# jseppanen/azalea

Measured on AMD Instinct MI355X. Metric: mcts_sims_per_sec, higher is better.
Workload: dtype f16x3 (fp32 operands split hi+lo f16, fp32 accumulate)

## Files before the change

azalea_amd/csrc/net_kernels.hip:

```cpp
#include "net_priv.h"

#ifndef AZX_NET_ABLATE
#define AZX_NET_ABLATE 0
#endif
#ifndef AZX_SAT_TRACK
#define AZX_SAT_TRACK 1
#endif

#include <cmath>
#include <cstdio>
#include <cstdlib>
#include <cstring>
#include <map>
#include <string>
#include <type_traits>
#include <vector>

typedef float f32x16 __attribute__((ext_vector_type(16)));

static thread_local std::string g_net_err;
const char *azx_net_error() { return g_net_err.c_str(); }

int azx_net_fail(int code, const char *msg) {
    g_net_err = msg;
// ... 99 lines not shown
                        acc[m][n] = __builtin_amdgcn_mfma_f32_32x32x2f32(afrag[m].y, bfrag[n].y, acc[m][n], 0, 0, 0);
                        acc[m][n] = __builtin_amdgcn_mfma_f32_32x32x2f32(afrag[m].z, bfrag[n].z, acc[m][n], 0, 0, 0);
                        acc[m][n] = __builtin_amdgcn_mfma_f32_32x32x2f32(afrag[m].w, bfrag[n].w, acc[m][n], 0, 0, 0);
                    }
            }
        }
        const bool residual = (layer & 1) != 0;
#pragma unroll
        for (int n = 0; n < NTW; ++n) {
            const int co = (ns * NTW + n) * 32 + li;
            const float bb = P.bias[layer * C + co];
#pragma unroll
            for (int m = 0; m < MTW; ++m) {
#pragma unroll
                for (int r = 0; r < 16; ++r) {
                    const int row = (ms * MTW + m) * 32 + (r & 3) + 8 * (r >> 2) + 4 * lh;
                    if (row < ncells) {
                        float v = acc[m][n][r] + bb;
                        if (residual) v += dst[row * LDW + co];
                        dst[row * LDW + co] = fmaxf(v, 0.0f);
                    }
                }
            }
        }
        __syncthreads();
    }

    for (int b = 0; b < BPB; ++b) {
        const int e = e0 + b;
        if (e >= n_eval) break;
        const float *Xb = lds + (size_t)b * 2 * rows * LDW;
        float4 *out = reinterpret_cast<float4 *>(act_out + (size_t)e * ncells * C);
        for (int idx = tid; idx < ncells * (C / 4); idx += 256) {
            const int pos = idx / (C / 4), c4 = idx - pos * (C / 4);
            out[idx] = *reinterpret_cast<const float4 *>(Xb + pos * LDW + 4 * c4);
        }
    }
}


typedef _Float16 f16x8 __attribute__((ext_vector_type(8)));

__device__ __forceinline__ void split_f16(float v, _Float16 &hi, _Float16 &lo) {
    hi = (_Float16)v;
    lo = (_Float16)(v - (float)hi);
}
__device__ __forceinline__ void split2_f16(float a, float b, uint32_t &hpk, uint32_t &lpk) {
    float la, lb;
    asm("v_cvt_pk_f16_f32 %0, %1, %2" : "=v"(hpk) : "v"(a), "v"(b));
    asm("v_fma_mix_f32 %0, %1, -1.0, %2 op_sel_hi:[1,0,0]" : "=v"(la) : "v"(hpk), "v"(a));
    asm("v_fma_mix_f32 %0, %1, -1.0, %2 op_sel:[1,0,0] op_sel_hi:[1,0,0]" : "=v"(lb) : "v"(hpk), "v"(b));
    asm("v_cvt_pk_f16_f32 %0, %1, %2" : "=v"(lpk) : "v"(la), "v"(lb));
#if AZX_LO_BITS < 10
    lpk = (lpk + LO_RND * 0x10001u) & (LO_MASK * 0x10001u);
#endif
}

#ifdef AZX_NET_STAMP
__device__ unsigned long long g_tower_stamp[10];
#define NT_DECL unsigned long long nt_last = __builtin_amdgcn_s_memtime(), nt_acc[8] = {0, 0, 0, 0, 0, 0, 0, 0}; const unsigned long long nt_rt0 = __builtin_amdgcn_s_memrealtime();
__device__ unsigned long long g_tower_trace[3 * 32768];
#define NT_MARK(r) { const unsigned long long nt_now = __builtin_amdgcn_s_memtime(); nt_acc[r] += nt_now - nt_last; nt_last = nt_now; }
#define NT_FLUSH if (tid == 0) { for (int r_ = 0; r_ < 7; ++r_) atomicAdd(&g_tower_stamp[r_], nt_acc[r_]); atomicAdd(&g_tower_stamp[7], 1ull); atomicAdd(&g_tower_stamp[8], __builtin_amdgcn_s_memrealtime() - nt_rt0); \
    if (blockIdx.x < 32768) { const unsigned hw = __builtin_amdgcn_s_getreg((31 << 11) | 4), xc = __builtin_amdgcn_s_getreg((31 << 11) | 20); \
        g_tower_trace[3 * blockIdx.x] = ((unsigned long long)(xc & 0xf) << 8) | (((hw >> 13) & 7) << 5) | (((hw >> 12) & 1) << 4) | ((hw >> 8) & 0xf); \
        g_tower_trace[3 * blockIdx.x + 1] = nt_rt0; g_tower_trace[3 * blockIdx.x + 2] = __builtin_amdgcn_s_memrealtime(); } }
__device__ unsigned long long g_wide_stamp[10];
#define WT_FLUSH if (lane == 0) { for (int r_ = 0; r_ < 7; ++r_) atomicAdd(&g_wide_stamp[r_], nt_acc[r_]); atomicAdd(&g_wide_stamp[7], 1ull); \
    atomicAdd(&g_wide_stamp[8], __builtin_amdgcn_s_memrealtime() - nt_rt0); }
#else
#define NT_DECL
#define NT_MARK(r)
#define NT_FLUSH
#define WT_FLUSH
#endif

#ifndef F16X3_BPB
#define F16X3_BPB 2
#endif
#ifndef AZX_S16_FENCE
#define AZX_S16_FENCE 1
#endif
typedef float f32x4 __attribute__((ext_vector_type(4)));

__global__ __launch_bounds__(F16X3_BPB * 128, 2) void k_tower_f16x3_s16(NetDev P, const uint8_t *__restrict__ ev_board,
                                                                        const int32_t *__restrict__ n_eval_ptr,
                                                                        int n_eval_host, float *__restrict__ act_out,
                                                                        float *__restrict__ hfeat) {
    constexpr int C = 64, ROWB = 272, MT = 4, NT = 4;
    extern __shared__ __align__(16) unsigned char smem[];
    const int n_eval = n_eval_ptr ? *n_eval_ptr : n_eval_host;
    const int e0 = blockIdx.x * F16X3_BPB;
    if (e0 >= n_eval) return;
    const int tid = threadIdx.x, lane = tid & 63, wave = __builtin_amdgcn_readfirstlane(tid >> 6);
    NT_DECL
    const int wb = wave >> 1, wh = wave & 1;
    const int N = P.N, ncells = P.ncells;
    const int e = e0 + wb;
    const bool live = e < n_eval;
    const int board_b = 128 * ROWB;
    const int zero_off = 0;
    const int x_off = 2 * ROWB + wb * board_b;
    unsigned char *X = smem + x_off;
    const int li = lane & 15, lh = lane >> 4;
    const int lrow = li < 8 ? li ^ 4 : li;
    const int lchunk = 128 * (lh & 1) + 16 * (lh >> 1);

    unsigned long long tapok = 0ull;
    int rbase[MT], ry_[MT], rx_[MT];
#pragma unroll
    for (int m = 0; m < MT; ++m) {
        const int r = 64 * wh + 16 * m + lrow;
        const int ry = r / N, rx = r - ry * N;
        ry_[m] = ry;
        rx_[m] = rx;
        rbase[m] = x_off + r * ROWB + lchunk;
#pragma unroll
        for (int tap = 0; tap < 9; ++tap) {
            const int yy = ry + tap / 3 - 1, xx = rx + tap % 3 - 1;
            if (r < ncells && yy >= 0 && yy < N && xx >= 0 && xx < N) tapok |= 1ull << (tap * 4 + m);
        }
    }
    uint32_t tapok_lo = (uint32_t)tapok, tapok_hi = (uint32_t)(tapok >> 32);
    auto act_offset = [&](int tap, int m) -> int {
        const int delta = ((tap / 3 - 1) * N + (tap % 3 - 1)) * ROWB;
        const uint32_t word = tap < 8 ? tapok_lo : tapok_hi;
        const int mask = (int)(word << (31 - ((tap * 4 + m) & 31))) >> 31;
        return (mask | 0xF0) & (rbase[m] + delta);
    };

    f32x4 res[MT][NT];
    auto load_bias = [&](const float *bias, float4 (&b4)[NT]) {
#pragma unroll
        for (int n = 0; n < NT; ++n) b4[n] = *reinterpret_cast<const float4 *>(bias + 16 * n + 4 * lh);
    };
    float satmax = 0.f;
    auto epilogue = [&](f32x4 (&acc)[MT][NT], const float4 (&bias4)[NT], auto kind_tag) {
        constexpr int kind = decltype(kind_tag)::value;
#pragma unroll
        for (int n = 0; n < NT; ++n) {
            const float4 b4 = bias4[n];
            const float bv[4] = {b4.x, b4.y, b4.z, b4.w};
#pragma unroll
            for (int m = 0; m < MT; ++m) {
                float v4[4];
#pragma unroll
                for (int j = 0; j < 4; ++j) {
                    float v = acc[m][n][j] + bv[j];
                    if (kind == 1) v += res[m][n][j];
                    v = fmaxf(v, 0.0f);
                    if (kind != 0) res[m][n][j] = v;
                    v4[j] = v;
                }
                if (AZX_SAT_TRACK) satmax = fmaxf(fmaxf(satmax, v4[0]), fmaxf(v4[1], fmaxf(v4[2], v4[3])));
                uint2 h4, l4;
                split2_f16(v4[0], v4[1], h4.x, l4.x);
                split2_f16(v4[2], v4[3], h4.y, l4.y);
                unsigned char *pw = X + (64 * wh + 16 * m + lrow) * ROWB + 128 * (lh >> 1) + 16 * n + 8 * (lh & 1);
                *reinterpret_cast<uint2 *>(pw) = h4;
                *reinterpret_cast<uint2 *>(pw + 64) = l4;
            }
        }
    };

    {
        const int NH = N + 2;
        unsigned char *cells = X + 121 * ROWB;
        const uint8_t *bd = ev_board + (size_t)(live ? e : n_eval - 1) * AZX_CELL_STRIDE;
        if (wh == 0) {
            for (int i = lane; i < NH * NH; i += 64) {
                const int y = i / NH - 1, x = i - (y + 1) * NH - 1;
                cells[i] = (y >= 0 && y < N && x >= 0 && x < N) ? bd[y * N + x] : (uint8_t)3;
            }
        }
        for (int i = tid; i < 2 * ROWB / 4; i += F16X3_BPB * 128) reinterpret_cast<uint32_t *>(smem + zero_off)[i] = 0u;
        __syncthreads();
        f32x4 acc[MT][NT];
#pragma unroll
        for (int m = 0; m < MT; ++m)
#pragma unroll
            for (int n = 0; n < NT; ++n) acc[m][n] = f32x4{0.f, 0.f, 0.f, 0.f};
        const uint4 *ws = reinterpret_cast<const uint4 *>(P.Ws16);
        f16x8 wfh[NT], wfl[NT];
#pragma unroll
        for (int n = 0; n < NT; ++n) {
            const uint4 qh = ws[(n * 2) * 64 + lane], ql = ws[(n * 2 + 1) * 64 + lane];
            wfh[n] = *reinterpret_cast<const f16x8 *>(&qh);
            wfl[n] = *reinterpret_cast<const f16x8 *>(&ql);
        }
#pragma unroll
        for (int m = 0; m < MT; ++m) {
            uint32_t onehot = 0u;
            if (64 * wh + 16 * m + lrow < ncells) {
                const unsigned char *c0 = cells + ry_[m] * NH + rx_[m];
#pragma unroll
                for (int tap = 0; tap < 9; ++tap) {
                    const uint32_t v = c0[(tap / 3) * NH + tap % 3];
                    onehot |= (v < 3u ? 1u : 0u) << (3 * tap + v);
                }
            }
            const uint32_t byte = (onehot >> (8 * lh)) & 0xffu;
            uint4 q;
            q.x = ((byte >> 0) & 1u) * 0x3C00u | ((byte >> 1) & 1u) * 0x3C000000u;
            q.y = ((byte >> 2) & 1u) * 0x3C00u | ((byte >> 3) & 1u) * 0x3C000000u;
            q.z = ((byte >> 4) & 1u) * 0x3C00u | ((byte >> 5) & 1u) * 0x3C000000u;
            q.w = ((byte >> 6) & 1u) * 0x3C00u | ((byte >> 7) & 1u) * 0x3C000000u;
            const f16x8 xf = *reinterpret_cast<const f16x8 *>(&q);
#pragma unroll
            for (int n = 0; n < NT; ++n) {
                acc[m][n] = __builtin_amdgcn_mfma_f32_16x16x32_f16(wfh[n], xf, acc[m][n], 0, 0, 0);
                acc[m][n] = __builtin_amdgcn_mfma_f32_16x16x32_f16(wfl[n], xf, acc[m][n], 0, 0, 0);
            }
        }
        float4 sb4[NT];
        load_bias(P.stem_b, sb4);
        __syncthreads();
        epilogue(acc, sb4, std::integral_constant<int, 2>{});
    }
    __syncthreads();
    NT_MARK(0)

    const uint4 *wsrc = reinterpret_cast<const uint4 *>(P.Wh16);
    int stage = 0;
    const int last_stage = P.layers * 18 - 1;
    f16x8 wh_[NT], wl_[NT];
    auto load_w = [&](int st, int nn, int part) {
        const uint4 qq = wsrc[(size_t)min(st, last_stage) * 512 + (nn * 2 + part) * 64 + lane];
        if (part) wl_[nn] = *reinterpret_cast<const f16x8 *>(&qq);
        else wh_[nn] = *reinterpret_cast<const f16x8 *>(&qq);
    };
#pragma unroll
    for (int i = 0; i < 4; ++i) load_w(0, i >> 1, i & 1);
    auto conv_layer = [&](int layer, auto residual_tag) {
        constexpr bool residual = decltype(residual_tag)::value;
        asm volatile("" : "+v"(tapok_lo), "+v"(tapok_hi), "+v"(rbase[0]), "+v"(rbase[1]), "+v"(rbase[2]), "+v"(rbase[3]));
        f32x4 acc[MT][NT];
#pragma unroll
        for (int m = 0; m < MT; ++m)
#pragma unroll
            for (int n = 0; n < NT; ++n) acc[m][n] = f32x4{0.f, 0.f, 0.f, 0.f};
        f16x8 xh[MT], xl[MT];
        auto load_x = [&](int tt, int mm, int part) {
            const unsigned char *pa = smem + act_offset(tt >> 1, mm) + (tt & 1) * 32 + part * 64;
            if (part) xl[mm] = *reinterpret_cast<const f16x8 *>(pa);
            else xh[mm] = *reinterpret_cast<const f16x8 *>(pa);
        };
#pragma unroll
        for (int m = 0; m < MT - 1; ++m) { load_x(0, m, 0); load_x(0, m, 1); }
#pragma unroll
        for (int t = 0; t < 18; ++t) {
#pragma unroll
            for (int h = 0; h < 2; ++h) {
#pragma unroll
                for (int q = 0; q < 24; ++q) {
                    const int m = q / 6, n = 2 * h + (q % 6) / 3, p = q % 3;
                    if (q == 1 || q == 4 || q == 7 || q == 10) {
                        const int idx = (q - 1) / 3;
                        if (h == 0) load_w(stage + t, 2 + (idx >> 1), idx & 1);
                        else load_w(stage + t + 1, idx >> 1, idx & 1);
                    } else if (h == 0 && (q == 13 || q == 16)) {
                        load_x(t, MT - 1, q == 16);
                    } else if (h == 1 && q >= 8 && (q % 6 == 2 || q % 6 == 5)) {
                        if (t + 1 < 18) load_x(t + 1, q / 6 - 1, q % 6 == 5);
                    }
                    const f16x8 wv = p == 1 ? wl_[n] : wh_[n];
                    const f16x8 xv = p == 2 ? xl[m] : xh[m];
                    acc[m][n] = __builtin_amdgcn_mfma_f32_16x16x32_f16(wv, xv, acc[m][n], 0, 0, 0);
#if AZX_S16_FENCE == 2
                    __builtin_amdgcn_sched_barrier(0);
#elif AZX_S16_FENCE == 1
                    if (q % 3 == 2) __builtin_amdgcn_sched_barrier(0);
#elif AZX_S16_FENCE == 3
                    if (q % 6 == 5) __builtin_amdgcn_sched_barrier(0);
#elif AZX_S16_FENCE == 4
                    if (q % 2 == 1) __builtin_amdgcn_sched_barrier(0);
#endif
                }
            }
        }
        stage += 18;
        float4 lb4[NT];
        load_bias(P.bias + layer * C, lb4);
        NT_MARK(2)
        __syncthreads();
        NT_MARK(3)
        epilogue(acc, lb4, std::integral_constant<int, residual ? 1 : 0>{});
        NT_MARK(4)
        __syncthreads();
        NT_MARK(5)
    };
    for (int blk = 0; blk < P.blocks; ++blk) {
        conv_layer(2 * blk, std::false_type{});
        conv_layer(2 * blk + 1, std::true_type{});
    }

    if (hfeat != nullptr) {
        const uint4 *whd = reinterpret_cast<const uint4 *>(P.Whd16);
        f16x8 ah[2], al[2];
#pragma unroll
        for (int ks = 0; ks < 2; ++ks) {
            const uint4 qh = whd[(ks * 2) * 64 + lane], ql = whd[(ks * 2 + 1) * 64 + lane];
            ah[ks] = *reinterpret_cast<const f16x8 *>(&qh);
            al[ks] = *reinterpret_cast<const f16x8 *>(&ql);
        }
        const float4 hb = *reinterpret_cast<const float4 *>(P.hbias16 + 4 * lh);
        const float hbv[4] = {hb.x, hb.y, hb.z, hb.w};
#pragma unroll
        for (int m = 0; m < MT; ++m) {
            f32x4 hacc = f32x4{0.f, 0.f, 0.f, 0.f};
#pragma unroll
            for (int ks = 0; ks < 2; ++ks) {
                const unsigned char *pa = smem + rbase[m] + ks * 32;
                const f16x8 xh = *reinterpret_cast<const f16x8 *>(pa), xl = *reinterpret_cast<const f16x8 *>(pa + 64);
                hacc = __builtin_amdgcn_mfma_f32_16x16x32_f16(ah[ks], xh, hacc, 0, 0, 0);
                hacc = __builtin_amdgcn_mfma_f32_16x16x32_f16(al[ks], xh, hacc, 0, 0, 0);
                hacc = __builtin_amdgcn_mfma_f32_16x16x32_f16(ah[ks], xl, hacc, 0, 0, 0);
            }
            const int row = 64 * wh + 16 * m + lrow;
            if (live && row < ncells) {
#pragma unroll
                for (int r = 0; r < 4; ++r) {
                    const int o = 4 * lh + r;
                    if (o < 6) hfeat[((size_t)e * 6 + o) * ncells + row] = fmaxf(hacc[r] + hbv[r], 0.0f);
                }
            }
        }
    }
    if (live && act_out != nullptr) {
        float *out = act_out + (size_t)e * ncells * C;
#pragma unroll
        for (int m = 0; m < MT; ++m) {
            const int row = 64 * wh + 16 * m + lrow;
            if (row < ncells) {
#pragma unroll
                for (int n = 0; n < NT; ++n)
                    *reinterpret_cast<float4 *>(out + row * C + 16 * n + 4 * lh) =
                        make_float4(res[m][n][0], res[m][n][1], res[m][n][2], res[m][n][3]);
            }
        }
    }
    if (satmax > 65504.0f) atomicOr(P.sat_flag, 1u);
    NT_MARK(6)
    NT_FLUSH
}

#define WIDE_ROWB 272
#define WIDE_MW 3
#define WIDE_NW 2

#ifndef WIDE_STAGE_GROUP
#define WIDE_STAGE_GROUP 6
#endif
#ifndef AZX_WIDE_ABLATE
#define AZX_WIDE_ABLATE 0
#endif

#define WIDE16_MT 6
#define WIDE16_NT 4
struct WideBwdFuse { const unsigned char *mask; const float *raw, *skip; const double *sums; float invN; unsigned int *gmax; };
template <int TRAIN, int NTW = WIDE16_NT>
__device__ __forceinline__ void conv_wide_s16_body(const NetDev &P, int layer, const unsigned short *__restrict__ in,
                                                   unsigned short *out, const unsigned short *resid,
                                                   float *__restrict__ out32,
                                                   const int32_t *__restrict__ n_eval_ptr, int n_eval_host,
                                                   int e_base, int e_end, float unscale, float2 *__restrict__ stat,
                                                   const WideBwdFuse &F = WideBwdFuse{}) {
    constexpr int MT = WIDE16_MT, NT = NTW, ROWB = WIDE_ROWB;
    static_assert(NT == 4 || (NT == 2 && TRAIN != 0), "two tiles per wave: training instantiations only");
    float satmax = 0.f;
    extern __shared__ __align__(16) unsigned char smem[];
    const int n_eval = n_eval_ptr ? *n_eval_ptr : n_eval_host;
    const int C = P.C, N = P.N, ncells = P.ncells;
    const int NCH = C / 64, NT16 = C / 16;
    NT_DECL
    const int e = e_base + blockIdx.y * 8 + (blockIdx.x & 7);
    if (e >= n_eval || e >= e_end) return;
    const int co_base = (blockIdx.x >> 3) * (32 * NT);
    const int tid = threadIdx.x, lane = tid & 63, wave = tid >> 6;
    const int wm = wave & 1, wn = wave >> 1;
    const int row0 = wm ? 80 : 0;
    const int li = lane & 15, lh = lane >> 4;
    const size_t rowg = (size_t)C * 4;
    const unsigned char *gin = reinterpret_cast<const unsigned char *>(in) + (size_t)e * ncells * rowg;
    constexpr int IMG0 = 2 * ROWB;
    const int lrow = li < 8 ? li ^ 4 : li;
    const int lchunk = 128 * (lh & 1) + 16 * (lh >> 1);

    unsigned long long tapok = 0ull;
    int rbase[MT];
#pragma unroll
    for (int m = 0; m < MT; ++m) {
        const int r = row0 + 16 * m + lrow;
        const int ry = r / N, rx = r - ry * N;
        rbase[m] = IMG0 + r * ROWB + lchunk;
#pragma unroll
        for (int tap = 0; tap < 9; ++tap) {
            const int yy = ry + tap / 3 - 1, xx = rx + tap % 3 - 1;
            if (r < ncells && yy >= 0 && yy < N && xx >= 0 && xx < N) tapok |= 1ull << (tap * 6 + m);
        }
    }
    uint32_t tapok_lo = (uint32_t)tapok & 0x3fffffffu, tapok_hi = (uint32_t)(tapok >> 30);
    auto act_offset = [&](int tap, int m) -> int {
        const int delta = ((tap / 3 - 1) * N + (tap % 3 - 1)) * ROWB;
        const uint32_t word = tap < 5 ? tapok_lo : tapok_hi;
        const int bit = (tap < 5 ? tap : tap - 5) * 6 + m;
        const int mask = (int)(word << (31 - bit)) >> 31;
        return (mask | 0xF0) & (rbase[m] + delta);
    };
    if (tid < IMG0 / 4) reinterpret_cast<uint32_t *>(smem)[tid] = 0u;

    auto chan0 = [&](int np) -> int { return co_base + 16 * NT * wn + 32 * np + 8 * lh; };
    f32x4 acc[MT][NT];
    if constexpr (TRAIN != 0) {
#pragma unroll
        for (int m = 0; m < MT; ++m)
#pragma unroll
            for (int n = 0; n < NT; ++n) acc[m][n] = f32x4{0.f, 0.f, 0.f, 0.f};
    } else {
        const unsigned char *gres0 = resid ? reinterpret_cast<const unsigned char *>(resid) + (size_t)e * ncells * rowg : nullptr;
#if AZX_WIDE_ABLATE & 16
        gres0 = nullptr;
#endif
        float bv[2][8];
#pragma unroll
        for (int np = 0; np < 2; ++np) {
            const float4 b0 = *reinterpret_cast<const float4 *>(P.bias + (size_t)layer * C + chan0(np));
// ... 828 lines not shown
                accm[4 * b4] += x.x * w; accm[4 * b4 + 1] += x.y * w; accm[4 * b4 + 2] += x.z * w; accm[4 * b4 + 3] += x.w * w;
            }
        }
    }
    if (HEADS_KSPLIT > 1) {
        if (part > 0) {
            float *ps = psum + (size_t)(part - 1) * (64 + 192) * HEADS_BPB;
#pragma unroll
            for (int b = 0; b < HEADS_BPB; ++b) {
                if (t < 64) ps[b * 64 + t] = acc2[b];
                if (t < ncells) ps[64 * HEADS_BPB + b * 192 + t] = accm[b];
            }
        }
        __syncthreads();
        if (part == 0) {
            for (int pp = 0; pp < HEADS_KSPLIT - 1; ++pp) {
                const float *ps = psum + (size_t)pp * (64 + 192) * HEADS_BPB;
#pragma unroll
                for (int b = 0; b < HEADS_BPB; ++b) {
                    if (t < 64) acc2[b] += ps[b * 64 + t];
                    if (t < ncells) accm[b] += ps[64 * HEADS_BPB + b * 192 + t];
                }
            }
        }
    }
    if (part == 0 && t < 64) {
#pragma unroll
        for (int b = 0; b < HEADS_BPB; ++b) h2[t][b] = fmaxf(acc2[b] + P.fc2b[t], 0.f);
    }
    if (part == 0 && t < ncells) {
        const float bias = P.mfcb[t];
#pragma unroll
        for (int b = 0; b < HEADS_BPB; ++b) {
            const float logit = accm[b] + bias;
            lg[b][t] = logit;
            if (b < nb) logit_out[(size_t)(e0 + b) * AZX_CELL_STRIDE + t] = logit;
        }
    }
    __syncthreads();
    if (tid < nb) {
        float acc = 0.f;
        for (int i = 0; i < 64; ++i) acc += h2[i][tid] * P.fc3w[i];
        value_out[e0 + tid] = tanhf(acc + P.fc3b[0]);
    }
    if (!prior_out) return;
    const int lane = tid & 63, wave = tid >> 6;
    for (int b = wave; b < nb; b += 3 * HEADS_KSPLIT) {
        const int e = e0 + b;
        float x[3];
        bool legal[3];
        float mx = -INFINITY;
#pragma unroll
        for (int s = 0; s < 3; ++s) {
            const int cell = s * 64 + lane;
            legal[s] = cell < ncells && ev_board[(size_t)e * AZX_CELL_STRIDE + cell] == 0;
            x[s] = legal[s] ? lg[b][cell] : -INFINITY;
            mx = fmaxf(mx, x[s]);
        }
        mx = wave_max(mx);
        float sum = 0.f;
#pragma unroll
        for (int s = 0; s < 3; ++s) sum += legal[s] ? expf(x[s] - mx) : 0.f;
        const float lse = mx + logf(wave_sum(sum));
        const int flip = ev_flip[e];
#pragma unroll
        for (int s = 0; s < 3; ++s) {
            const int cell = s * 64 + lane;
            if (cell < ncells) {
                int oc = cell;
                if (flip) {
                    const int i = cell / N, j = cell - i * N;
                    oc = (N - 1 - j) * N + (N - 1 - i);
                }
                prior_out[(size_t)e * AZX_CELL_STRIDE + oc] = legal[s] ? expf(x[s] - lse) : 0.f;
            }
        }
    }
}



static int raise_lds_limits() {
    const int cap = 160 * 1024;
    const void *fns[] = {(const void *)k_tower_f16x3_s16, (const void *)k_conv_wide_f16x3_s16,
                         (const void *)k_tower_mfma<64, 4, 2, 1, 2>, (const void *)k_tower_mfma<64, 6, 1, 2, 2>,
                         (const void *)k_tower_mfma<32, 6, 2, 2, 1>, (const void *)k_heads_mfma, (const void *)k_heads};
    for (const void *f : fns)
        if (hipFuncSetAttribute(f, hipFuncAttributeMaxDynamicSharedMemorySize, cap) != hipSuccess)
            return nfail(AZX_EHIP, "net: raising a tower kernel's dynamic LDS limit failed");
    return AZX_OK;
}

int azx_net_create(AzxNet **out, int N, int blocks, int chans, int max_evals, hipStream_t st) {
    if (N < 2 || N > AZX_MAX_BOARD) return nfail(AZX_EINVAL, "net: board size out of range");
    if (blocks < 0 || chans < 1) return nfail(AZX_EINVAL, "net: bad num_blocks/base_chans");
    if (int rc = raise_lds_limits()) return rc;
    AzxNet *net = new AzxNet();
    memset(&net->d, 0, sizeof net->d);
    net->d.N = N;
    net->d.ncells = N * N;
    net->d.C = chans;
    net->d.blocks = blocks;
    net->d.layers = 2 * blocks;
    net->max_evals = max_evals;
    net->stream = st;
    const int ncells = N * N;
    const char *force = getenv("AZX_TOWER");
    const bool want_fp32 = force && !strcmp(force, "fp32");
    if (chans == 64 && ncells <= 121 && blocks >= 1 && !want_fp32) net->tower_variant = 4;
    else if (chans == 64 && ncells <= 128) net->tower_variant = 1;
    else if (chans == 64 && ncells <= 192) net->tower_variant = 2;
    else if (chans == 32 && ncells <= 192) net->tower_variant = 3;
    else if (chans % 128 == 0 && ncells <= 192 && !want_fp32) net->tower_variant = 5;
    net->use_mfma = net->tower_variant != 0;
    { const char *v = getenv("AZX_WIDE_STREAMS"); net->opt_wsplit = std::min(4, std::max(1, v ? atoi(v) : 2)); }
    { const char *v = getenv("AZX_HEADS"); net->opt_heads_mfma = !(v && !strcmp(v, "valu")); }
    { const char *v = getenv("AZX_PACK"); net->pack_on_host = v && !strcmp(v, "host"); }
    {
        char b[260];
        const char *tower = "k_stem_generic + k_conv_generic (VALU)";
        if (net->tower_variant == 4) tower = "k_tower_f16x3_s16";
        else if (net->tower_variant == 5) tower = "k_stem_wide_f16x3 + k_conv_wide_f16x3_s16 per layer";
        else if (net->tower_variant == 1) tower = "k_tower_mfma<64,4,2,1,2> (fp32 MFMA)";
        else if (net->tower_variant == 2) tower = "k_tower_mfma<64,6,1,2,2> (fp32 MFMA)";
        else if (net->tower_variant == 3) tower = "k_tower_mfma<32,6,2,2,1> (fp32 MFMA)";
        const bool hm = net->tower_variant == 4 && net->opt_heads_mfma && ncells <= 128;
        snprintf(b, sizeof b, "%s + %s (%dx%d on %dx%d; AZX_TOWER=%s AZX_WIDE_STREAMS=%d AZX_HEADS=%s AZX_PACK=%s)",
                 tower, hm ? "k_heads_mfma" : "k_heads", blocks, chans, N, N, want_fp32 ? "fp32" : "default",
                 net->opt_wsplit, net->opt_heads_mfma ? "mfma" : "valu", net->pack_on_host ? "host" : "device");
        net->info = b;
    }
    const size_t E = max_evals;
    net->act = nalloc<float>(net, E * ncells * chans);
    net->logit = nalloc<float>(net, E * AZX_CELL_STRIDE);
    if (net->tower_variant == 4) net->hfeat = nalloc<float>(net, E * 6 * ncells);
    net->hb_board = nalloc<uint8_t>(net, E * AZX_CELL_STRIDE);
    net->hb_flip = nalloc<int32_t>(net, E);
    net->hb_value = nalloc<float>(net, E);
    if (!net->use_mfma) {
        net->act2 = nalloc<float>(net, E * ncells * chans);
        net->act3 = nalloc<float>(net, E * ncells * chans);
    }
    if (net->tower_variant == 5) {
        net->wideX = nalloc<unsigned short>(net, E * ncells * chans * 2);
        net->wideY = nalloc<unsigned short>(net, E * ncells * chans * 2);
    }
    if (!net->act || !net->logit || !net->hb_board || !net->hb_flip || !net->hb_value ||
        (!net->use_mfma && (!net->act2 || !net->act3)) || (net->tower_variant == 5 && (!net->wideX || !net->wideY))) {
        azx_net_destroy(net);
        return nfail(AZX_ENOMEM, "net: hipMalloc failed");
    }
    const int bpb = net->tower_variant == 2 ? 1 : 2;
    net->lds_bytes = (size_t)bpb * 2 * (ncells + 1) * (chans + 4) * sizeof(float);
    if (net->tower_variant == 4) net->lds_bytes = (size_t)F16X3_BPB * 128 * 272 + 2 * 272;
    if (net->tower_variant == 5) net->lds_bytes = (size_t)(ncells + 2) * WIDE_ROWB;
    net->d.sat_flag = nalloc<uint32_t>(net, 4);
    if (!net->d.sat_flag || hipDeviceSynchronize() != hipSuccess) {
        azx_net_destroy(net);
        return nfail(AZX_ENOMEM, "net: hipMalloc failed");
    }
    *out = net;
    return AZX_OK;
}

void azx_net_set_stream(AzxNet *net, hipStream_t st, const uint32_t *mask, int words) {
    if (!net) return;
    for (int i = 0; i < 3; ++i) {
        if (net->stream2[i]) { (void)hipStreamSynchronize(net->stream2[i]); (void)hipStreamDestroy(net->stream2[i]); }
        if (net->ev_join[i]) (void)hipEventDestroy(net->ev_join[i]);
        net->stream2[i] = nullptr;
        net->ev_join[i] = nullptr;
    }
    if (net->ev_fork) (void)hipEventDestroy(net->ev_fork);
    net->ev_fork = nullptr;
    net->streams_ok = false;
    net->cu_mask.assign(mask, mask + (mask ? words : 0));
    net->stream = st;
}

void azx_net_destroy(AzxNet *net) {
    if (net) {
        for (int i = 0; i < 3; ++i) {
            if (net->stream2[i]) { (void)hipStreamSynchronize(net->stream2[i]); (void)hipStreamDestroy(net->stream2[i]); }
            if (net->ev_join[i]) (void)hipEventDestroy(net->ev_join[i]);
            net->stream2[i] = nullptr;
            net->ev_join[i] = nullptr;
        }
        if (net->ev_fork) (void)hipEventDestroy(net->ev_fork);
        net->ev_fork = nullptr;
    }
#ifdef AZX_NET_STAMP
    {
        unsigned long long h[10] = {0};
        if (hipMemcpyFromSymbol(h, HIP_SYMBOL(g_wide_stamp), sizeof h) == hipSuccess && h[7]) {
            static const char *nm[6] = {"prologue (bias + residual, setup)", "barrier after staging", "k-loops (MFMA)", "epilogue (stores acknowledged)",
                                        "barrier before staging (skew)", "staging: requests, round trips, LDS writes"};
            unsigned long long tot = 0;
            for (int r = 0; r < 6; ++r) tot += h[r];
            fprintf(stderr, "k_conv_wide_f16x3_s16 stamps over %llu waves: %.0f cycles/wave, shader clock %.0f MHz during the kernel\n",
                    h[7], (double)tot / h[7], h[8] ? 100.0 * (double)tot / (double)h[8] : 0.0);
            for (int r = 0; r < 6; ++r)
                fprintf(stderr, "  %-44s %6.1f%%  %9.0f cycles/wave\n", nm[r], 100.0 * h[r] / tot, (double)h[r] / h[7]);
            unsigned long long z[10] = {0};
            (void)hipMemcpyToSymbol(HIP_SYMBOL(g_wide_stamp), z, sizeof z);
        }
    }
    {
        unsigned long long h[10] = {0};
        if (hipMemcpyFromSymbol(h, HIP_SYMBOL(g_tower_stamp), sizeof h) == hipSuccess && h[7]) {
            static const char *nm[7] = {"stem", "residual load/setup", "k-loop (MFMA)", "barrier after k-loop",
                                        "epilogue", "barrier after epilogue", "output store"};
            unsigned long long tot = 0;
            for (int r = 0; r < 7; ++r) tot += h[r];
            fprintf(stderr, "k_tower_f16x3_s16 stamps over %llu blocks: %.0f cycles/block, shader clock %.0f MHz during the kernel\n",
                    h[7], (double)tot / h[7], h[8] ? 100.0 * (double)tot / (double)h[8] : 0.0);
            for (int r = 0; r < 7; ++r)
                fprintf(stderr, "  %-24s %6.1f%%  %9.0f cycles/block\n", nm[r], 100.0 * h[r] / tot, (double)h[r] / h[7]);
            {
                std::vector<unsigned long long> tr(3 * 32768);
                (void)hipMemcpyFromSymbol(tr.data(), HIP_SYMBOL(g_tower_trace), tr.size() * sizeof(unsigned long long));
                std::map<unsigned long long, std::vector<std::pair<unsigned long long, unsigned long long>>> cu;
                unsigned long long t0 = ~0ull, t1 = 0;
                size_t nblk = 0;
                for (int b = 0; b < 32768; ++b)
                    if (tr[3 * b + 2]) {
                        cu[tr[3 * b]].push_back({tr[3 * b + 1], tr[3 * b + 2]});
                        t0 = std::min(t0, tr[3 * b + 1]);
                        t1 = std::max(t1, tr[3 * b + 2]);
                        ++nblk;
                    }
                double busy = 0, mn = 1e30, mx = 0, lastend_min = 1e30, lastend_max = 0;
                size_t cmin = 1 << 30, cmax = 0;
                for (auto &kv : cu) {
                    double b = 0, le = 0;
                    for (auto &iv : kv.second) { b += (double)(iv.second - iv.first); le = std::max(le, (double)(iv.second - t0)); }
                    busy += b; mn = std::min(mn, b); mx = std::max(mx, b);
                    cmin = std::min(cmin, kv.second.size()); cmax = std::max(cmax, kv.second.size());
                    lastend_min = std::min(lastend_min, le); lastend_max = std::max(lastend_max, le);
                }
                fprintf(stderr, "  last launch: %zu blocks on %zu CUs, span %.1f us, blocks/CU %zu..%zu, mean resident blocks/CU %.2f, "
                        "per-CU block-time %.0f..%.0f us, CU finish %.0f..%.0f us\n", nblk, cu.size(), (t1 - t0) / 100.0, cmin, cmax,
                        busy / ((double)(t1 - t0) * cu.size()), mn / 100.0, mx / 100.0, lastend_min / 100.0, lastend_max / 100.0);
            }
            int nb = -1;
            (void)hipOccupancyMaxActiveBlocksPerMultiprocessor(&nb, (const void *)k_tower_f16x3_s16, F16X3_BPB * 128, net->lds_bytes);
            hipFuncAttributes fa;
            memset(&fa, 0, sizeof fa);
            (void)hipFuncGetAttributes(&fa, (const void *)k_tower_f16x3_s16);
            fprintf(stderr, "  runtime occupancy: %d blocks/CU (dynamic LDS %zu B, static %zu B, %d VGPRs, max threads %d)\n", nb,
                    net->lds_bytes, (size_t)fa.sharedSizeBytes, fa.numRegs, fa.maxThreadsPerBlock);
        }
    }
#endif
    if (!net) return;
    for (void *p : net->allocs) (void)hipFree(p);
    if (net->raw_tab_host) (void)hipHostFree((void *)net->raw_tab_host);
    if (net->wmax_host) (void)hipHostFree((void *)net->wmax_host);
    delete net;
}

bool azx_net_ready(const AzxNet *net) { return net && net->ready; }


static void run_net(AzxNet *net, const uint8_t *boards, const int32_t *flip, const int32_t *n_eval_ptr,
                    int n_host, int max_n, float *logit, float *value, float *prior, hipStream_t st, size_t row0 = 0) {
    const NetDev &d = net->d;
    if (max_n <= 0) return;
    const size_t act_rows = row0 * d.ncells * d.C;
    float *const act = net->act + act_rows;
    float *const act2 = net->act2 ? net->act2 + act_rows : nullptr;
    float *const act3 = net->act3 ? net->act3 + act_rows : nullptr;
    float *const hfeat_rows = net->hfeat ? net->hfeat + row0 * 6 * d.ncells : nullptr;
    const float *hfeat = nullptr;
    if (net->use_mfma) {
        const size_t lds = net->lds_bytes;
        if (net->tower_variant == 4) {
            const dim3 grid((max_n + F16X3_BPB - 1) / F16X3_BPB), block(F16X3_BPB * 128);
            hipLaunchKernelGGL(k_tower_f16x3_s16, grid, block, lds, st, d, boards, n_eval_ptr, n_host, (float *)nullptr, hfeat_rows);
            hfeat = hfeat_rows;
        } else if (net->tower_variant == 5) {
            const dim3 grid(max_n, d.C / 128), block(256);
            hipLaunchKernelGGL(k_stem_wide_f16x3, grid, block, 0, st, d, boards, net->wideX,
                               d.blocks == 0 ? net->act : (float *)nullptr, n_eval_ptr, n_host);
            const int wsplit = net->opt_wsplit;
            {
                int parts = wsplit;
                if (parts > 1 && !net->ev_fork) {
                    bool ok = hipEventCreateWithFlags(&net->ev_fork, hipEventDisableTiming) == hipSuccess;
                    for (int i = 0; i < 3 && ok; ++i)
                        ok = (net->cu_mask.empty() ? hipStreamCreateWithFlags(&net->stream2[i], hipStreamNonBlocking)
                                                   : hipExtStreamCreateWithCUMask(&net->stream2[i], (uint32_t)net->cu_mask.size(), net->cu_mask.data())) == hipSuccess &&
                             hipEventCreateWithFlags(&net->ev_join[i], hipEventDisableTiming) == hipSuccess;
                    net->streams_ok = ok;
                }
                if (parts > 1 && !net->streams_ok) parts = 1;
                const int per = (((max_n + parts - 1) / parts + 7) / 8) * 8;
                if (per >= max_n) parts = 1;
                if (parts > 1 && hipEventRecord(net->ev_fork, st) != hipSuccess) parts = 1;
                for (int part = 1; part < parts; ++part)
                    if (hipStreamWaitEvent(net->stream2[part - 1], net->ev_fork, 0) != hipSuccess) { parts = 1; break; }
                const int per_ok = parts > 1 ? per : max_n;
                for (int part = 0; part < parts; ++part) {
                    hipStream_t s = part ? net->stream2[part - 1] : st;
                    const int e0 = part * per_ok, e1 = std::min(max_n, e0 + per_ok);
                    if (e1 <= e0) continue;
                    const dim3 g(8 * (d.C / 128), (e1 - e0 + 7) / 8);
                    for (int b = 0; b < d.blocks; ++b) {
                        hipLaunchKernelGGL(k_conv_wide_f16x3_s16, g, block, lds, s, d, 2 * b, (const unsigned short *)net->wideX, net->wideY,
                                           (const unsigned short *)nullptr, (float *)nullptr, n_eval_ptr, n_host, e0, e1);
                        hipLaunchKernelGGL(k_conv_wide_f16x3_s16, g, block, lds, s, d, 2 * b + 1, (const unsigned short *)net->wideY, net->wideX,
                                           (const unsigned short *)net->wideX, b == d.blocks - 1 ? net->act : (float *)nullptr, n_eval_ptr, n_host, e0, e1);
                    }
                    if (part) {
                        if (hipEventRecord(net->ev_join[part - 1], s) != hipSuccess ||
                            hipStreamWaitEvent(st, net->ev_join[part - 1], 0) != hipSuccess)
                            (void)hipStreamSynchronize(s);
                    }
                }
            }
        } else if (net->tower_variant == 1) {
            hipLaunchKernelGGL((k_tower_mfma<64, 4, 2, 1, 2>), dim3((max_n + 1) / 2), dim3(256), lds, st, d, boards, n_eval_ptr, n_host, act);
        } else if (net->tower_variant == 2) {
            hipLaunchKernelGGL((k_tower_mfma<64, 6, 1, 2, 2>), dim3(max_n), dim3(256), lds, st, d, boards, n_eval_ptr, n_host, act);
        } else {
            hipLaunchKernelGGL((k_tower_mfma<32, 6, 2, 2, 1>), dim3((max_n + 1) / 2), dim3(256), lds, st, d, boards, n_eval_ptr, n_host, act);
        }
    } else {
        const int grid = 2048;
        hipLaunchKernelGGL(k_stem_generic, dim3(grid), dim3(256), 0, st, d, boards, n_eval_ptr, n_host, act);
        float *x = act, *y = act2, *z = act3;
        for (int b = 0; b < d.blocks; ++b) {
            hipLaunchKernelGGL(k_conv_generic, dim3(grid), dim3(256), 0, st, d, 2 * b, x, (const float *)nullptr, n_eval_ptr, n_host, y);
            hipLaunchKernelGGL(k_conv_generic, dim3(grid), dim3(256), 0, st, d, 2 * b + 1, y, x, n_eval_ptr, n_host, z);
            std::swap(x, z);
        }
        if (x != act)
            (void)hipMemcpyAsync(act, x, (size_t)max_n * d.ncells * d.C * sizeof(float), hipMemcpyDeviceToDevice, st);
    }
    if (hfeat != nullptr && net->opt_heads_mfma && d.ncells <= 128) {
        const size_t hl = std::max((size_t)HM_MB * d.hm_lda, (size_t)HM_MB * AZX_CELL_STRIDE + (size_t)HM_MB * 64) * sizeof(float);
        hipLaunchKernelGGL(k_heads_mfma, dim3((max_n + HM_MB - 1) / HM_MB), dim3(256), hl, st, d, hfeat, boards, flip, n_eval_ptr, n_host, logit, value, prior);
    } else {
        const size_t hl = ((size_t)(6 * d.ncells + 64) * HEADS_BPB + (size_t)HEADS_BPB * AZX_CELL_STRIDE +
                           (size_t)(HEADS_KSPLIT - 1) * (64 + 192) * HEADS_BPB) * sizeof(float);
        hipLaunchKernelGGL(k_heads, dim3((max_n + HEADS_BPB - 1) / HEADS_BPB), dim3(192 * HEADS_KSPLIT), hl, st, d, act, hfeat, boards, flip, n_eval_ptr, n_host, logit, value, prior);
    }
}

const char *azx_net_kernel_info(const AzxNet *net) { return net->info.c_str(); }

int azx_net_check_range(AzxNet *net, hipStream_t st) {
    if (!net || !net->d.sat_flag) return AZX_OK;
    uint32_t flag = 0;
    if (hipMemcpyAsync(&flag, net->d.sat_flag, sizeof flag, hipMemcpyDeviceToHost, st) != hipSuccess ||
        hipStreamSynchronize(st) != hipSuccess)
        return nfail(AZX_EHIP, "net: reading the activation range flag failed");
    if (!flag) return AZX_OK;
    (void)hipMemsetAsync(net->d.sat_flag, 0, sizeof flag, st);
    return nfail(AZX_ERANGE, "net: an activation of the residual tower exceeded the f16 range (65504) of the split-f16 "
                             "kernels -- the evaluations of this call are not valid (AZX_TOWER=fp32 runs the fp32 MFMA tower)");
}
// ... 58 lines not shown
```

Baseline: 5.253 million.

## Template f16x3 tower on board size with zero-padded halo LDS layout and buffer loads

Templates the f16x3 tower kernel on board size N so cell counts and strides are compile-time constants. It replaces the per-tap validity bitmask and masked offset computation with a zero-padded (N+1)-row halo layout in LDS, so every tap reads directly and out-of-board neighbours hit zeros. Weight and bias loads go through buffer resource descriptors with scalar offsets, and the epilogue is vectorised per row using packed f32x2 adds. The cost is ten kernel instantiations, extra LDS zeroing of the halo bands, and dispatch through a function table.

Result: no change. 5.254 million, median of 3 (+0.0%).

```diff
diff --git a/azalea_amd/csrc/net_kernels.hip b/azalea_amd/csrc/net_kernels.hip
--- a/azalea_amd/csrc/net_kernels.hip
+++ b/azalea_amd/csrc/net_kernels.hip
@@ -205,12 +205,30 @@
 #define AZX_S16_FENCE 1
 #endif
 typedef float f32x4 __attribute__((ext_vector_type(4)));
-
+typedef float f32x2 __attribute__((ext_vector_type(2)));
+typedef unsigned int u32x4 __attribute__((ext_vector_type(4)));
+
+#define F16X3_ROWB 272
+__host__ __device__ constexpr int f16x3_lds_bytes(int N) {
+    return F16X3_BPB * (N + 1) * ((N + 1) * F16X3_ROWB - 16) + (N + 1) * F16X3_ROWB + 256;
+}
+
+__device__ __forceinline__ f16x8 wfrag(__amdgpu_buffer_rsrc_t r, int voff, int soff, int f) {
+    const u32x4 q = __builtin_amdgcn_raw_buffer_load_b128(r, voff + (f & 3) * 1024, soff + (f >> 2) * 4096, 0);
+    return __builtin_bit_cast(f16x8, q);
+}
+__device__ __forceinline__ __amdgpu_buffer_rsrc_t wrsrc(const void *p, int bytes) {
+    return __builtin_amdgcn_make_buffer_rsrc(const_cast<void *>(p), (short)0, bytes, 0x00020000);
+}
+
+template <int N>
 __global__ __launch_bounds__(F16X3_BPB * 128, 2) void k_tower_f16x3_s16(NetDev P, const uint8_t *__restrict__ ev_board,
                                                                         const int32_t *__restrict__ n_eval_ptr,
                                                                         int n_eval_host, float *__restrict__ act_out,
                                                                         float *__restrict__ hfeat) {
-    constexpr int C = 64, ROWB = 272, MT = 4, NT = 4;
+    constexpr int C = 64, ROWB = F16X3_ROWB, MT = 4, NT = 4;
+    constexpr int ncells = N * N;
+    constexpr int BRP = (N + 1) * ROWB - 16, BST = (N + 1) * BRP;
     extern __shared__ __align__(16) unsigned char smem[];
     const int n_eval = n_eval_ptr ? *n_eval_ptr : n_eval_host;
     const int e0 = blockIdx.x * F16X3_BPB;
@@ -218,77 +236,84 @@
     const int tid = threadIdx.x, lane = tid & 63, wave = __builtin_amdgcn_readfirstlane(tid >> 6);
     NT_DECL
     const int wb = wave >> 1, wh = wave & 1;
-    const int N = P.N, ncells = P.ncells;
     const int e = e0 + wb;
     const bool live = e < n_eval;
-    const int board_b = 128 * ROWB;
-    const int zero_off = 0;
-    const int x_off = 2 * ROWB + wb * board_b;
-    unsigned char *X = smem + x_off;
     const int li = lane & 15, lh = lane >> 4;
     const int lrow = li < 8 ? li ^ 4 : li;
     const int lchunk = 128 * (lh & 1) + 16 * (lh >> 1);
 
-    unsigned long long tapok = 0ull;
     int rbase[MT], ry_[MT], rx_[MT];
+    bool cell[MT];
 #pragma unroll
     for (int m = 0; m < MT; ++m) {
         const int r = 64 * wh + 16 * m + lrow;
-        const int ry = r / N, rx = r - ry * N;
+        cell[m] = r < ncells;
+        const int p = min(r, ncells - 1);
+        const int ry = p / N, rx = p - ry * N;
         ry_[m] = ry;
         rx_[m] = rx;
-        rbase[m] = x_off + r * ROWB + lchunk;
-#pragma unroll
-        for (int tap = 0; tap < 9; ++tap) {
-            const int yy = ry + tap / 3 - 1, xx = rx + tap % 3 - 1;
-            if (r < ncells && yy >= 0 && yy < N && xx >= 0 && xx < N) tapok |= 1ull << (tap * 4 + m);
-        }
-    }
-    uint32_t tapok_lo = (uint32_t)tapok, tapok_hi = (uint32_t)(tapok >> 32);
-    auto act_offset = [&](int tap, int m) -> int {
-        const int delta = ((tap / 3 - 1) * N + (tap % 3 - 1)) * ROWB;
-        const uint32_t word = tap < 8 ? tapok_lo : tapok_hi;
-        const int mask = (int)(word << (31 - ((tap * 4 + m) & 31))) >> 31;
-        return (mask | 0xF0) & (rbase[m] + delta);
-    };
+        rbase[m] = wb * BST + ry * BRP + rx * ROWB + lchunk;
+    }
+    constexpr auto tap_off = [](int tap) { return (tap / 3) * BRP + (tap % 3) * ROWB; };
+    const int wdelta = tap_off(4) + 128 * (lh >> 1) + 8 * (lh & 1) - lchunk;
 
     f32x4 res[MT][NT];
-    auto load_bias = [&](const float *bias, float4 (&b4)[NT]) {
-#pragma unroll
-        for (int n = 0; n < NT; ++n) b4[n] = *reinterpret_cast<const float4 *>(bias + 16 * n + 4 * lh);
+    const __amdgpu_buffer_rsrc_t brs = wrsrc(P.bias, P.layers * C * 4);
+    const int boff = 16 * lh;
+    auto load_bias = [&](__amdgpu_buffer_rsrc_t r, int soff, float4 (&b4)[NT]) {
+#pragma unroll
+        for (int n = 0; n < NT; ++n)
+            b4[n] = __builtin_bit_cast(float4, __builtin_amdgcn_raw_buffer_load_b128(r, boff, soff + 64 * n, 0));
     };
     float satmax = 0.f;
     auto epilogue = [&](f32x4 (&acc)[MT][NT], const float4 (&bias4)[NT], auto kind_tag) {
         constexpr int kind = decltype(kind_tag)::value;
 #pragma unroll
-        for (int n = 0; n < NT; ++n) {
-            const float4 b4 = bias4[n];
-            const float bv[4] = {b4.x, b4.y, b4.z, b4.w};
-#pragma unroll
-            for (int m = 0; m < MT; ++m) {
-                float v4[4];
-#pragma unroll
-                for (int j = 0; j < 4; ++j) {
-                    float v = acc[m][n][j] + bv[j];
-                    if (kind == 1) v += res[m][n][j];
-                    v = fmaxf(v, 0.0f);
-                    if (kind != 0) res[m][n][j] = v;
-                    v4[j] = v;
-                }
-                if (AZX_SAT_TRACK) satmax = fmaxf(fmaxf(satmax, v4[0]), fmaxf(v4[1], fmaxf(v4[2], v4[3])));
-                uint2 h4, l4;
-                split2_f16(v4[0], v4[1], h4.x, l4.x);
-                split2_f16(v4[2], v4[3], h4.y, l4.y);
-                unsigned char *pw = X + (64 * wh + 16 * m + lrow) * ROWB + 128 * (lh >> 1) + 16 * n + 8 * (lh & 1);
-                *reinterpret_cast<uint2 *>(pw) = h4;
-                *reinterpret_cast<uint2 *>(pw + 64) = l4;
+        for (int m = 0; m < MT; ++m) {
+            uint2 h4[NT], l4[NT];
+            float mx = 0.f;
+#pragma unroll
+            for (int n = 0; n < NT; ++n) {
+                const float4 b4 = bias4[n];
+                f32x2 v01 = f32x2{acc[m][n][0], acc[m][n][1]} + f32x2{b4.x, b4.y};
+                f32x2 v23 = f32x2{acc[m][n][2], acc[m][n][3]} + f32x2{b4.z, b4.w};
+                if (kind == 1) {
+                    v01 += f32x2{res[m][n][0], res[m][n][1]};
+                    v23 += f32x2{res[m][n][2], res[m][n][3]};
+                }
+                const float v4[4] = {fmaxf(v01.x, 0.0f), fmaxf(v01.y, 0.0f), fmaxf(v23.x, 0.0f), fmaxf(v23.y, 0.0f)};
+                if (kind != 0) res[m][n] = f32x4{v4[0], v4[1], v4[2], v4[3]};
+                if (AZX_SAT_TRACK) mx = fmaxf(fmaxf(mx, v4[0]), fmaxf(v4[1], fmaxf(v4[2], v4[3])));
+                split2_f16(v4[0], v4[1], h4[n].x, l4[n].x);
+                split2_f16(v4[2], v4[3], h4[n].y, l4[n].y);
+            }
+            if (cell[m]) {
+                if (AZX_SAT_TRACK) satmax = fmaxf(satmax, mx);
+                unsigned char *pw = smem + rbase[m] + wdelta;
+#pragma unroll
+                for (int n = 0; n < NT; ++n) {
+                    *reinterpret_cast<uint2 *>(pw + 16 * n) = h4[n];
+                    *reinterpret_cast<uint2 *>(pw + 16 * n + 64) = l4[n];
+                }
             }
         }
     };
 
     {
-        const int NH = N + 2;
-        unsigned char *cells = X + 121 * ROWB;
+        constexpr int BAND = ((N + 1) * ROWB + 256) / 16, ZBLK = ROWB / 16;
+        constexpr int NZ = (F16X3_BPB + 1) * BAND + F16X3_BPB * (N - 1) * ZBLK;
+        for (int i = tid; i < NZ; i += F16X3_BPB * 128) {
+            int off;
+            if (i < (F16X3_BPB + 1) * BAND) {
+                off = (i / BAND) * BST + 16 * (i % BAND);
+            } else {
+                const int k = i - (F16X3_BPB + 1) * BAND, z = k / ZBLK;
+                off = (z / (N - 1)) * BST + (z % (N - 1) + 2) * BRP + 16 * (k % ZBLK);
+            }
+            *reinterpret_cast<uint4 *>(smem + off) = uint4{0u, 0u, 0u, 0u};
+        }
+        constexpr int NH = N + 2;
+        unsigned char *cells = smem + wb * BST + BRP + ROWB;
         const uint8_t *bd = ev_board + (size_t)(live ? e : n_eval - 1) * AZX_CELL_STRIDE;
         if (wh == 0) {
             for (int i = lane; i < NH * NH; i += 64) {
@@ -296,31 +321,27 @@
                 cells[i] = (y >= 0 && y < N && x >= 0 && x < N) ? bd[y * N + x] : (uint8_t)3;
             }
         }
-        for (int i = tid; i < 2 * ROWB / 4; i += F16X3_BPB * 128) reinterpret_cast<uint32_t *>(smem + zero_off)[i] = 0u;
         __syncthreads();
         f32x4 acc[MT][NT];
 #pragma unroll
         for (int m = 0; m < MT; ++m)
 #pragma unroll
             for (int n = 0; n < NT; ++n) acc[m][n] = f32x4{0.f, 0.f, 0.f, 0.f};
-        const uint4 *ws = reinterpret_cast<const uint4 *>(P.Ws16);
+        const __amdgpu_buffer_rsrc_t wsr = wrsrc(P.Ws16, 8 * 1024);
         f16x8 wfh[NT], wfl[NT];
 #pragma unroll
         for (int n = 0; n < NT; ++n) {
-            const uint4 qh = ws[(n * 2) * 64 + lane], ql = ws[(n * 2 + 1) * 64 + lane];
-            wfh[n] = *reinterpret_cast<const f16x8 *>(&qh);
-            wfl[n] = *reinterpret_cast<const f16x8 *>(&ql);
+            wfh[n] = wfrag(wsr, 16 * lane, 0, n * 2);
+            wfl[n] = wfrag(wsr, 16 * lane, 0, n * 2 + 1);
         }
 #pragma unroll
         for (int m = 0; m < MT; ++m) {
             uint32_t onehot = 0u;
-            if (64 * wh + 16 * m + lrow < ncells) {
-                const unsigned char *c0 = cells + ry_[m] * NH + rx_[m];
-#pragma unroll
-                for (int tap = 0; tap < 9; ++tap) {
-                    const uint32_t v = c0[(tap / 3) * NH + tap % 3];
-                    onehot |= (v < 3u ? 1u : 0u) << (3 * tap + v);
-                }
+            const unsigned char *c0 = cells + ry_[m] * NH + rx_[m];
+#pragma unroll
+            for (int tap = 0; tap < 9; ++tap) {
+                const uint32_t v = c0[(tap / 3) * NH + tap % 3];
+                onehot |= (v < 3u ? 1u : 0u) << (3 * tap + v);
             }
             const uint32_t byte = (onehot >> (8 * lh)) & 0xffu;
             uint4 q;
@@ -336,27 +357,29 @@
             }
         }
         float4 sb4[NT];
-        load_bias(P.stem_b, sb4);
+        load_bias(wrsrc(P.stem_b, C * 4), 0, sb4);
         __syncthreads();
         epilogue(acc, sb4, std::integral_constant<int, 2>{});
     }
     __syncthreads();
     NT_MARK(0)
 
-    const uint4 *wsrc = reinterpret_cast<const uint4 *>(P.Wh16);
+    const __amdgpu_buffer_rsrc_t wres = wrsrc(P.Wh16, P.layers * 18 * 8192);
+    const int voff = 16 * lane;
     int stage = 0;
     const int last_stage = P.layers * 18 - 1;
     f16x8 wh_[NT], wl_[NT];
+    int vo = voff;
     auto load_w = [&](int st, int nn, int part) {
-        const uint4 qq = wsrc[(size_t)min(st, last_stage) * 512 + (nn * 2 + part) * 64 + lane];
-        if (part) wl_[nn] = *reinterpret_cast<const f16x8 *>(&qq);
-        else wh_[nn] = *reinterpret_cast<const f16x8 *>(&qq);
+        const f16x8 q = wfrag(wres, vo, min(st, last_stage) * 8192, nn * 2 + part);
+        if (part) wl_[nn] = q;
+        else wh_[nn] = q;
     };
 #pragma unroll
     for (int i = 0; i < 4; ++i) load_w(0, i >> 1, i & 1);
     auto conv_layer = [&](int layer, auto residual_tag) {
         constexpr bool residual = decltype(residual_tag)::value;
-        asm volatile("" : "+v"(tapok_lo), "+v"(tapok_hi), "+v"(rbase[0]), "+v"(rbase[1]), "+v"(rbase[2]), "+v"(rbase[3]));
+        asm volatile("" : "+v"(vo));
         f32x4 acc[MT][NT];
 #pragma unroll
         for (int m = 0; m < MT; ++m)
@@ -364,7 +387,7 @@
             for (int n = 0; n < NT; ++n) acc[m][n] = f32x4{0.f, 0.f, 0.f, 0.f};
         f16x8 xh[MT], xl[MT];
         auto load_x = [&](int tt, int mm, int part) {
-            const unsigned char *pa = smem + act_offset(tt >> 1, mm) + (tt & 1) * 32 + part * 64;
+            const unsigned char *pa = smem + rbase[mm] + tap_off(tt >> 1) + (tt & 1) * 32 + part * 64;
             if (part) xl[mm] = *reinterpret_cast<const f16x8 *>(pa);
             else xh[mm] = *reinterpret_cast<const f16x8 *>(pa);
         };
@@ -403,7 +426,7 @@
         }
         stage += 18;
         float4 lb4[NT];
-        load_bias(P.bias + layer * C, lb4);
+        load_bias(brs, layer * C * 4, lb4);
         NT_MARK(2)
         __syncthreads();
         NT_MARK(3)
@@ -418,13 +441,12 @@
     }
 
     if (hfeat != nullptr) {
-        const uint4 *whd = reinterpret_cast<const uint4 *>(P.Whd16);
+        const __amdgpu_buffer_rsrc_t hrs = wrsrc(P.Whd16, 4 * 1024);
         f16x8 ah[2], al[2];
 #pragma unroll
         for (int ks = 0; ks < 2; ++ks) {
-            const uint4 qh = whd[(ks * 2) * 64 + lane], ql = whd[(ks * 2 + 1) * 64 + lane];
-            ah[ks] = *reinterpret_cast<const f16x8 *>(&qh);
-            al[ks] = *reinterpret_cast<const f16x8 *>(&ql);
+            ah[ks] = wfrag(hrs, voff, 0, ks * 2);
+            al[ks] = wfrag(hrs, voff, 0, ks * 2 + 1);
         }
         const float4 hb = *reinterpret_cast<const float4 *>(P.hbias16 + 4 * lh);
         const float hbv[4] = {hb.x, hb.y, hb.z, hb.w};
@@ -433,14 +455,14 @@
             f32x4 hacc = f32x4{0.f, 0.f, 0.f, 0.f};
 #pragma unroll
             for (int ks = 0; ks < 2; ++ks) {
-                const unsigned char *pa = smem + rbase[m] + ks * 32;
+                const unsigned char *pa = smem + rbase[m] + tap_off(4) + ks * 32;
                 const f16x8 xh = *reinterpret_cast<const f16x8 *>(pa), xl = *reinterpret_cast<const f16x8 *>(pa + 64);
                 hacc = __builtin_amdgcn_mfma_f32_16x16x32_f16(ah[ks], xh, hacc, 0, 0, 0);
                 hacc = __builtin_amdgcn_mfma_f32_16x16x32_f16(al[ks], xh, hacc, 0, 0, 0);
                 hacc = __builtin_amdgcn_mfma_f32_16x16x32_f16(ah[ks], xl, hacc, 0, 0, 0);
             }
             const int row = 64 * wh + 16 * m + lrow;
-            if (live && row < ncells) {
+            if (live && cell[m]) {
 #pragma unroll
                 for (int r = 0; r < 4; ++r) {
                     const int o = 4 * lh + r;
@@ -454,7 +476,7 @@
 #pragma unroll
         for (int m = 0; m < MT; ++m) {
             const int row = 64 * wh + 16 * m + lrow;
-            if (row < ncells) {
+            if (cell[m]) {
 #pragma unroll
                 for (int n = 0; n < NT; ++n)
                     *reinterpret_cast<float4 *>(out + row * C + 16 * n + 4 * lh) =
@@ -465,6 +487,23 @@
     if (satmax > 65504.0f) atomicOr(P.sat_flag, 1u);
     NT_MARK(6)
     NT_FLUSH
+}
+
+typedef void (*F16x3TowerFn)(NetDev, const uint8_t *, const int32_t *, int, float *, float *);
+static F16x3TowerFn f16x3_tower(int N) {
+    switch (N) {
+        case 2: return k_tower_f16x3_s16<2>;
+        case 3: return k_tower_f16x3_s16<3>;
+        case 4: return k_tower_f16x3_s16<4>;
+        case 5: return k_tower_f16x3_s16<5>;
+        case 6: return k_tower_f16x3_s16<6>;
+        case 7: return k_tower_f16x3_s16<7>;
+        case 8: return k_tower_f16x3_s16<8>;
+        case 9: return k_tower_f16x3_s16<9>;
+        case 10: return k_tower_f16x3_s16<10>;
+        case 11: return k_tower_f16x3_s16<11>;
+    }
+    return nullptr;
 }
 
 #define WIDE_ROWB 272
@@ -1459,9 +1498,10 @@
 
 static int raise_lds_limits() {
     const int cap = 160 * 1024;
-    const void *fns[] = {(const void *)k_tower_f16x3_s16, (const void *)k_conv_wide_f16x3_s16,
-                         (const void *)k_tower_mfma<64, 4, 2, 1, 2>, (const void *)k_tower_mfma<64, 6, 1, 2, 2>,
-                         (const void *)k_tower_mfma<32, 6, 2, 2, 1>, (const void *)k_heads_mfma, (const void *)k_heads};
+    std::vector<const void *> fns = {(const void *)k_conv_wide_f16x3_s16,
+                                     (const void *)k_tower_mfma<64, 4, 2, 1, 2>, (const void *)k_tower_mfma<64, 6, 1, 2, 2>,
+                                     (const void *)k_tower_mfma<32, 6, 2, 2, 1>, (const void *)k_heads_mfma, (const void *)k_heads};
+    for (int n = 2; n <= 11; ++n) fns.push_back((const void *)f16x3_tower(n));
     for (const void *f : fns)
         if (hipFuncSetAttribute(f, hipFuncAttributeMaxDynamicSharedMemorySize, cap) != hipSuccess)
             return nfail(AZX_EHIP, "net: raising a tower kernel's dynamic LDS limit failed");
@@ -1529,7 +1569,7 @@
     }
     const int bpb = net->tower_variant == 2 ? 1 : 2;
     net->lds_bytes = (size_t)bpb * 2 * (ncells + 1) * (chans + 4) * sizeof(float);
-    if (net->tower_variant == 4) net->lds_bytes = (size_t)F16X3_BPB * 128 * 272 + 2 * 272;
+    if (net->tower_variant == 4) net->lds_bytes = (size_t)f16x3_lds_bytes(N);
     if (net->tower_variant == 5) net->lds_bytes = (size_t)(ncells + 2) * WIDE_ROWB;
     net->d.sat_flag = nalloc<uint32_t>(net, 4);
     if (!net->d.sat_flag || hipDeviceSynchronize() != hipSuccess) {
@@ -1620,10 +1660,10 @@
                         busy / ((double)(t1 - t0) * cu.size()), mn / 100.0, mx / 100.0, lastend_min / 100.0, lastend_max / 100.0);
             }
             int nb = -1;
-            (void)hipOccupancyMaxActiveBlocksPerMultiprocessor(&nb, (const void *)k_tower_f16x3_s16, F16X3_BPB * 128, net->lds_bytes);
+            (void)hipOccupancyMaxActiveBlocksPerMultiprocessor(&nb, (const void *)f16x3_tower(net->d.N), F16X3_BPB * 128, net->lds_bytes);
             hipFuncAttributes fa;
             memset(&fa, 0, sizeof fa);
-            (void)hipFuncGetAttributes(&fa, (const void *)k_tower_f16x3_s16);
+            (void)hipFuncGetAttributes(&fa, (const void *)f16x3_tower(net->d.N));
             fprintf(stderr, "  runtime occupancy: %d blocks/CU (dynamic LDS %zu B, static %zu B, %d VGPRs, max threads %d)\n", nb,
                     net->lds_bytes, (size_t)fa.sharedSizeBytes, fa.numRegs, fa.maxThreadsPerBlock);
         }
@@ -1653,7 +1693,7 @@
         const size_t lds = net->lds_bytes;
         if (net->tower_variant == 4) {
             const dim3 grid((max_n + F16X3_BPB - 1) / F16X3_BPB), block(F16X3_BPB * 128);
-            hipLaunchKernelGGL(k_tower_f16x3_s16, grid, block, lds, st, d, boards, n_eval_ptr, n_host, (float *)nullptr, hfeat_rows);
+            hipLaunchKernelGGL(f16x3_tower(d.N), grid, block, lds, st, d, boards, n_eval_ptr, n_host, (float *)nullptr, hfeat_rows);
             hfeat = hfeat_rows;
         } else if (net->tower_variant == 5) {
             const dim3 grid(max_n, d.C / 128), block(256);
```
